# rampasek/DrVAE

Hardware: AMD Instinct MI355X
Metric: DrVAE ELBO training samples/sec (batch x L) (higher is better)
Workload: dtype f32; 1 GPU; cfg2: DrVAE bortezomib shape: 978 genes, z1=z3=100, enc-z1 800, dec-x 600, enc-z3/dec-z1 200, batch 150/GPU, L=2; global_batch=150, L=2, parallelism=dp1, launch=hipGraph replay, feed=resident, side_chain_cus=64, rccl_ranks=0, params=2321758

## Files before the change

### drvae_amd/csrc/rows.hip

```cpp
#include "dv_common.h"

namespace {

constexpr float kLog2Pi = 1.8378770664093453f;

inline int grid_for(int64_t work, int per_block, int cap = 4096) {
    int64_t b = (work + per_block - 1) / per_block;
    if (b < 1) b = 1;
    if (b > cap) b = cap;
    return (int)b;
}

__global__ __launch_bounds__(256) void colsum_kernel(const float* __restrict__ X, int64_t ldx, int M, int N,
                                                     float* __restrict__ out, float beta) {
    __shared__ float part[4][64];
    const int c = threadIdx.x & 63, rl = threadIdx.x >> 6;
    const int col = blockIdx.x * 64 + c;
    float s = 0.f;
    if (col < N) {
        const float* p = X + (int64_t)rl * ldx + col;
        const int64_t st = 4 * ldx;
        int m = rl;
        float a0 = 0.f, a1 = 0.f, a2 = 0.f, a3 = 0.f, a4 = 0.f, a5 = 0.f, a6 = 0.f, a7 = 0.f;
        for (; m + 28 < M; m += 32, p += 8 * st) {
            const float v0 = p[0], v1 = p[st], v2 = p[2 * st], v3 = p[3 * st];
            const float v4 = p[4 * st], v5 = p[5 * st], v6 = p[6 * st], v7 = p[7 * st];
            a0 += v0; a1 += v1; a2 += v2; a3 += v3;
            a4 += v4; a5 += v5; a6 += v6; a7 += v7;
        }
        s = ((a0 + a1) + (a2 + a3)) + ((a4 + a5) + (a6 + a7));
        for (; m < M; m += 4, p += st) s += p[0];
    }
    part[rl][c] = s;
    __syncthreads();
    if (rl == 0 && col < N) {
        s = part[0][c] + part[1][c] + part[2][c] + part[3][c];
        out[col] = (beta != 0.f ? beta * out[col] : 0.f) + s;
    }
}

__global__ void act_bwd_kernel(float* __restrict__ dY, int64_t ldd, const float* __restrict__ Y, int64_t ldy, int M,
                               int N, int split, int act0, int act1, float shift0, float shift1) {
    const int64_t total = (int64_t)M * N;
    for (int64_t e = blockIdx.x * (int64_t)blockDim.x + threadIdx.x; e < total; e += (int64_t)gridDim.x * blockDim.x) {
        const int m = (int)(e / N), n = (int)(e % N);
        const bool first = n < split;
        const float y = Y[(int64_t)m * ldy + n] - (first ? shift0 : shift1);
        dY[(int64_t)m * ldd + n] *= dv_dact_from_y(first ? act0 : act1, y);
    }
}

__global__ __launch_bounds__(256) void wn_scale_kernel(const float* __restrict__ W, int64_t ldw,
                                                       const float* __restrict__ g, int N, int K,
                                                       float* __restrict__ scale, float* __restrict__ norm) {
    const int lane = threadIdx.x & 63;
    const int row = blockIdx.x * 4 + (threadIdx.x >> 6);
    if (row >= N) return;
    const float* w = W + (int64_t)row * ldw;
    float s = 0.f;
    for (int k = lane; k < K; k += 64) s += w[k] * w[k];
    s = dv_wave_sum_all(s);
    if (lane == 0) {
        const float nrm = sqrtf(s);
        if (norm) norm[row] = nrm;
        scale[row] = g[row] / nrm;
    }
}

__global__ __launch_bounds__(256) void wn_bwd_kernel(const float* __restrict__ dWraw, int64_t ldr,
                                                     const float* __restrict__ W, int64_t ldw,
                                                     const float* __restrict__ g, const float* __restrict__ norm,
                                                     int N, int K, float* __restrict__ dW, int64_t ldd,
                                                     float* __restrict__ dg, float beta) {
    const int lane = threadIdx.x & 63;
    const int row = blockIdx.x * 4 + (threadIdx.x >> 6);
    if (row >= N) return;
    const float* w = W + (int64_t)row * ldw;
    const float* r = dWraw + (int64_t)row * ldr;
    float dot = 0.f;
    for (int k = lane; k < K; k += 64) dot += w[k] * r[k];
    dot = dv_wave_sum_all(dot);
    const float nrm = norm[row], gg = g[row];
    const float sc = gg / nrm, cw = dot * gg / (nrm * nrm * nrm);
    float* o = dW + (int64_t)row * ldd;
    for (int k = lane; k < K; k += 64) {
        const float v = sc * r[k] - cw * w[k];
        o[k] = (beta != 0.f ? beta * o[k] : 0.f) + v;
    }
    if (lane == 0) dg[row] = (beta != 0.f ? beta * dg[row] : 0.f) + dot / nrm;
}

__global__ void reparam_fwd_kernel(const float* __restrict__ mu, const float* __restrict__ sd, int64_t ldq,
                                   const int32_t* __restrict__ src_idx, int n, int reps, int Z,
                                   const float* __restrict__ eps, int64_t lde, int mode, float* __restrict__ out,
                                   int64_t ldo, const float* __restrict__ sub, int64_t lds,
                                   float* __restrict__ out2, int64_t ldo2, float* __restrict__ out3, int64_t ldo3,
                                   const int32_t* __restrict__ out3_idx) {
    const int64_t total = (int64_t)n * reps * Z;
    for (int64_t e = blockIdx.x * (int64_t)blockDim.x + threadIdx.x; e < total; e += (int64_t)gridDim.x * blockDim.x) {
        const int r = (int)(e / Z), d = (int)(e % Z);
        const int j = r % n;
        const int64_t qi = src_idx ? src_idx[j] : j;
        const float s = sd[qi * ldq + d];
        const float std_ = mode == DV_GAUSS_LOGVAR ? expf(0.5f * s) : s;
        const float z = eps[(int64_t)r * lde + d] * std_ + mu[qi * ldq + d];
        out[(int64_t)r * ldo + d] = z;
        if (out2) out2[(int64_t)r * ldo2 + d] = z - sub[(int64_t)r * lds + d];
        if (out3) {
            const int t = out3_idx[r];
            if (t >= 0) out3[(int64_t)t * ldo3 + d] = z;
        }
    }
}

__global__ void reparam_bwd_kernel(const float* __restrict__ dz, int64_t ldz, const float* __restrict__ eps,
                                   int64_t lde, const float* __restrict__ sd, int64_t ldq,
                                   const int32_t* __restrict__ src_idx, int n, int reps, int Z, int mode,
                                   float* __restrict__ dmu, float* __restrict__ dsd, int64_t lddq, float beta) {
    const int64_t total = (int64_t)n * Z;
    for (int64_t e = blockIdx.x * (int64_t)blockDim.x + threadIdx.x; e < total; e += (int64_t)gridDim.x * blockDim.x) {
        const int j = (int)(e / Z), d = (int)(e % Z);
        const int64_t qi = src_idx ? src_idx[j] : j;
        float a = 0.f, b = 0.f;
        for (int l = 0; l < reps; ++l) {
            const int64_t r = (int64_t)l * n + j;
            const float g = dz[r * ldz + d];
            a += g;
            b += g * eps[r * lde + d];
        }
        if (mode == DV_GAUSS_LOGVAR) b *= 0.5f * expf(0.5f * sd[qi * ldq + d]);
        float* pm = dmu + qi * lddq + d;
        float* ps = dsd + qi * lddq + d;
        *pm = (beta != 0.f ? beta * *pm : 0.f) + a;
        *ps = (beta != 0.f ? beta * *ps : 0.f) + b;
    }
}

#define DV_MAX_PARKED_GRID 512
typedef dv_wait ParkArgs;
typedef dv_bump CounterBump;

__device__ __forceinline__ void bump_counters(const CounterBump& bump) {
    for (int t = 0; t < 2; ++t) {
        if (bump.c[t] != nullptr) counter_add_words(bump.c[t], bump.n[t], bump.inc[t]);
    }
}

__device__ __forceinline__ float free_bits_gate(float c, float rv, float kl_min) {
    return c * (rv > kl_min ? 1.f : (rv == kl_min ? 0.5f : 0.f));
}

struct KlGrad {
    float gmq, gsq, gmp, gsp;
};
__device__ __forceinline__ KlGrad kl_grad_logvar(float mq, float sq, float mp, float sp) {
    const float dm = mq - mp, ivp = expf(-sp), vq = expf(sq);
    KlGrad g;
    g.gmq = dm * ivp;
    g.gsq = -0.5f * (1.f - vq * ivp);
    g.gmp = -g.gmq;
    g.gsp = -0.5f * (-1.f + (dm * dm + vq) * ivp);
    return g;
}

__global__ void reparam_bwd_seg_kernel(const float* __restrict__ dz, int64_t ldz, const float* __restrict__ eps,
                                       int64_t lde, const float* __restrict__ sd, int64_t ldq,
                                       const int32_t* __restrict__ seg_ptr, const int32_t* __restrict__ seg_rows,
                                       int nq, int Z, int mode, const float* __restrict__ extra, int64_t ldx,
                                       const int32_t* __restrict__ ex_ptr, const int32_t* __restrict__ ex_rows,
                                       float* __restrict__ dmu, float* __restrict__ dsd, int64_t lddq, float beta,
                                       CounterBump bump, const float* __restrict__ dz2, int64_t ldz2, int n2,
                                       ParkArgs park, dv_prior_kl pk) {
    park_block(park);
    if (blockIdx.x == 0 && threadIdx.x == 0) bump_counters(bump);
    const int64_t total = (int64_t)nq * Z;
    for (int64_t e = blockIdx.x * (int64_t)blockDim.x + threadIdx.x; e < total; e += (int64_t)gridDim.x * blockDim.x) {
        const int i = (int)(e / Z), d = (int)(e % Z);
        float a = 0.f, b = 0.f;
        for (int t = seg_ptr[i]; t < seg_ptr[i + 1]; ++t) {
            const int64_t r = seg_rows[t];
            float g = dz[r * ldz + d];
            if (r < n2) g += dz2[r * ldz2 + d];
            a += g;
            b += g * eps[r * lde + d];
        }
        if (mode == DV_GAUSS_LOGVAR) b *= 0.5f * expf(0.5f * sd[(int64_t)i * ldq + d]);
        if (extra) {
            for (int t = ex_ptr[i]; t < ex_ptr[i + 1]; ++t) {
                const int64_t r = ex_rows[t];
                a += extra[r * ldx + d];
                b += extra[r * ldx + Z + d];
            }
        }
        float* pm = dmu + (int64_t)i * lddq + d;
        float* ps = dsd + (int64_t)i * lddq + d;
        float vm = (beta != 0.f ? beta * *pm : 0.f) + a;
        float vs = (beta != 0.f ? beta * *ps : 0.f) + b;
        if (pk.coef != nullptr) {
            const float c = free_bits_gate(pk.coef[i], pk.raw[i], pk.kl_min);
            const float mq = pk.mu[(int64_t)i * pk.ld + d], vq = expf(sd[(int64_t)i * ldq + d]);
            vm += c * (mq * 1.f);
            vs += c * (-0.5f * (1.f - vq * 1.f));
        }
        *pm = vm;
        *ps = vs;
    }
}

struct Z2FArgs {
    const float* dz2f; int64_t ld_dz2f;
    const float* dzdec_pert; int64_t ld_pert;
    const int32_t* pair_slot;
    const float* eps; int64_t lde;
    const float* p2; int64_t ldp2;
    const float* q2; int64_t ldq2;
    const float* coef; const float* raw; float kl_min;
    const float* dz1b; int64_t ld_dz1b;
    float* dp2; int64_t ld_dp2;
    float* dz1; int64_t ld_dz1;
    float* dq2; int64_t ld_dq2;
    int L, B, Np, Z;
    const float* prior_coef; const float* prior_raw;
    float* kl_out; float* raw_out;
    const float* seg_src; int64_t ld_seg; const int32_t* seg_ptr; float seg_beta;
    float z1_dz2f;
};

__device__ __forceinline__ float kl_term(int mode, float mq, float sq, float mp, float sp) {
    const float dm = mq - mp;
    if (mode == DV_GAUSS_LOGVAR) return 1.f - sp + sq - (dm * dm + expf(sq)) / expf(sp);
    const float vq = sq * sq, vp = sp * sp;
    return 1.f - logf(vp) + logf(vq) - (dm * dm + vq) / vp;
}

struct Z2FElem {
    float mp, lp, gc, g, eps, z1, add;
};

__device__ __forceinline__ void z2f_load_own(const Z2FArgs& a, int64_t r, int64_t kr, int d, Z2FElem& e) {
    e.mp = a.p2[r * a.ldp2 + d];
    e.lp = a.p2[r * a.ldp2 + a.Z + d];
    e.g = (kr >= 0 && a.dzdec_pert) ? a.dzdec_pert[kr * a.ld_pert + d] : 0.f;
    e.eps = a.eps[r * a.lde + d];
    e.z1 = a.dz1[r * a.ld_dz1 + d];
}

__device__ __forceinline__ void z2f_load_side(const Z2FArgs& a, int64_t r, int d, int t0, int t1, Z2FElem& e) {
    e.gc = a.dz2f ? a.dz2f[r * a.ld_dz2f + d] : 0.f;
    e.g = e.gc + e.g;
    e.add = a.dz1b ? a.dz1b[r * a.ld_dz1b + d] : 0.f;
    if (a.seg_src != nullptr) {
        float s = 0.f;
        for (int t = t0; t < t1; ++t) s += a.seg_src[(int64_t)t * a.ld_seg + d];
        e.add += a.seg_beta * s;
    }
    if (a.z1_dz2f != 0.f) e.add += a.z1_dz2f * e.gc;
}

__device__ __forceinline__ void z2f_elem(const Z2FArgs& a, int64_t r, int d, bool pair, float c, float mq, float lq,
                                         const Z2FElem& e, float& gq_mu, float& gq_lv) {
    float dmu = e.g, dlv = e.g * e.eps * 0.5f * expf(0.5f * e.lp);
    if (pair) {
        const float dm = mq - e.mp, ivp = expf(-e.lp);
        const KlGrad k = kl_grad_logvar(mq, lq, e.mp, e.lp);
        gq_mu += c * dm * ivp;
        gq_lv += c * k.gsq;
        dmu += -c * dm * ivp;
        dlv += c * k.gsp;
    }
    a.dp2[r * a.ld_dp2 + d] = dmu;
    a.dp2[r * a.ld_dp2 + a.Z + d] = dlv;
    a.dz1[r * a.ld_dz1 + d] = e.z1 + (dmu + e.add);
}

struct Z2FRow {
    int jp;
    bool pair, own_kl, prior;
    float cpr, mq[2], lq[2], gm[2], gl[2];
};
struct Z2FPair {
    Z2FElem e[2][2];
    int t0[2], t1[2];
    float cf[2], rv[2];
};

__device__ __forceinline__ void z2f_row_begin(const Z2FArgs& a, int i, int lane, Z2FRow& w) {
    w.jp = a.pair_slot ? a.pair_slot[i] : -1;
    w.pair = w.jp >= 0;
    w.own_kl = w.pair && a.raw_out != nullptr;
    w.prior = w.pair && a.dq2 && a.prior_coef != nullptr;
    w.cpr = 0.f;
    if (w.prior)
        w.cpr = free_bits_gate(a.prior_coef[w.jp], a.prior_raw[w.jp], a.kl_min);
#pragma unroll
    for (int c = 0; c < 2; ++c) {
        const int d = lane + 64 * c;
        w.mq[c] = w.lq[c] = w.gm[c] = w.gl[c] = 0.f;
        if (w.pair && d < a.Z) {
            w.mq[c] = a.q2[(int64_t)w.jp * a.ldq2 + d];
            w.lq[c] = a.q2[(int64_t)w.jp * a.ldq2 + a.Z + d];
        }
    }
}

__device__ __forceinline__ void z2f_pair_own(const Z2FArgs& a, const Z2FRow& w, int i, int l0, int lane, Z2FPair& g) {
#pragma unroll
    for (int u = 0; u < 2; ++u) {
        g.t0[u] = g.t1[u] = 0;
        g.cf[u] = g.rv[u] = 0.f;
        if (l0 + u >= a.L) break;
        const int64_t r = (int64_t)(l0 + u) * a.B + i, kr = w.pair ? (int64_t)(l0 + u) * a.Np + w.jp : -1;
        if (a.seg_src != nullptr) {
            g.t0[u] = a.seg_ptr[r];
            g.t1[u] = a.seg_ptr[r + 1];
        }
        if (w.pair) g.cf[u] = a.coef[kr];
#pragma unroll
        for (int c = 0; c < 2; ++c)
            if (lane + 64 * c < a.Z) z2f_load_own(a, r, kr, lane + 64 * c, g.e[u][c]);
    }
    if (!w.own_kl) return;
#pragma unroll
    for (int u = 0; u < 2; ++u) {
        if (l0 + u >= a.L) break;
        float s = 0.f;
#pragma unroll
        for (int c = 0; c < 2; ++c)
            if (lane + 64 * c < a.Z) s += kl_term(DV_GAUSS_LOGVAR, w.mq[c], w.lq[c], g.e[u][c].mp, g.e[u][c].lp);
        g.rv[u] = -0.5f * dv_wave_sum_all(s);
        if (lane == 0) {
            const int64_t kr = (int64_t)(l0 + u) * a.Np + w.jp;
            a.raw_out[kr] = g.rv[u];
            a.kl_out[kr] = fmaxf(g.rv[u], a.kl_min);
        }
    }
}

__device__ __forceinline__ void z2f_pair_finish(const Z2FArgs& a, Z2FRow& w, int i, int l0, int lane, Z2FPair& g) {
#pragma unroll
    for (int u = 0; u < 2; ++u) {
        if (l0 + u >= a.L) break;
        const int64_t r = (int64_t)(l0 + u) * a.B + i;
        if (w.pair && !w.own_kl) g.rv[u] = a.raw[(int64_t)(l0 + u) * a.Np + w.jp];
#pragma unroll
        for (int c = 0; c < 2; ++c)
            if (lane + 64 * c < a.Z) z2f_load_side(a, r, lane + 64 * c, g.t0[u], g.t1[u], g.e[u][c]);
    }
#pragma unroll
    for (int u = 0; u < 2; ++u) {
        if (l0 + u >= a.L) break;
        const int64_t r = (int64_t)(l0 + u) * a.B + i;
        const float cg = w.pair ? free_bits_gate(g.cf[u], g.rv[u], a.kl_min) : 0.f;
#pragma unroll
        for (int c = 0; c < 2; ++c)
            if (lane + 64 * c < a.Z)
                z2f_elem(a, r, lane + 64 * c, w.pair, cg, w.mq[c], w.lq[c], g.e[u][c], w.gm[c], w.gl[c]);
    }
}
// ... 2408 lines not shown
                    for (; j + 3 < rl; j += 4) {
                        s0 += xr[j];
                        s1 += xr[j + 1];
                        s2 += xr[j + 2];
                        s3 += xr[j + 3];
                    }
                    for (; j < rl; ++j) s0 += xr[j];
                    q += t.w[r] * ((s0 + s1) + (s2 + s3));
                }
            } else {
                for (int i = threadIdx.x; i < t.n; i += kLossThreads) q += t.x[i];
            }
            ps[k] = q;
        }
    }
#pragma unroll
    for (int k = 0; k < DV_MAX_LOSS_TERMS; ++k) {
        if (k >= lt.n) continue;
        const float q = dv_wave_sum_all(ps[k]);
        if ((threadIdx.x & 63) == 0) part[k][threadIdx.x >> 6] = q;
    }
    __syncthreads();
    if (threadIdx.x == 0) {
        for (int i = 0; i < 8; ++i) acc[i] = 0.f;
        for (int k = 0; k < lt.n; ++k) {
            float q = 0.f;
            for (int w = 0; w < kLossThreads / 64; ++w) q += part[k][w];
            acc[lt.t[k].out] += lt.t[k].scale * q;
        }
    }
    if (threadIdx.x == 0) {
        if (!(flag != nullptr && lt.n == 0)) {
            acc[5] = we[0] * acc[0] + we[1] * acc[1] + we[2] * acc[2];
            float c = 0.f;
#pragma unroll
            for (int i = 0; i < 8; ++i) c += wc[i] * acc[i];
            acc[6] = c;
            bool bad = false;
            for (int i = 0; i < n_halt; ++i)
                bad = bad || __hip_atomic_load(halt + 2 * i, __ATOMIC_RELAXED, __HIP_MEMORY_SCOPE_AGENT) != 0;
            for (int i = 0; i < 8; ++i) loss[i] = bad ? __builtin_nanf("") : acc[i];
            if (accum != nullptr) {
#pragma unroll
                for (int i = 0; i < 8; ++i) accum[i] = ac[i] + (bad ? __builtin_nanf("") : acc[i]);
            }
        }
        bump_counters(bump);
    }
}

__global__ void axpby_kernel(const float* __restrict__ x, float a, float* __restrict__ y, float b, int64_t n) {
    for (int64_t i = blockIdx.x * (int64_t)blockDim.x + threadIdx.x; i < n; i += (int64_t)gridDim.x * blockDim.x)
        y[i] = a * x[i] + (b != 0.f ? b * y[i] : 0.f);
}

inline bool aligned16(const void* p) { return (reinterpret_cast<uintptr_t>(p) & 15) == 0; }

}

#define ST(s) static_cast<hipStream_t>(s)

static bool park_ok(const dv_wait* p) { return p == nullptr || p->flag == nullptr || (p->ctr && p->err && p->max_spins > 0); }
static bool bump_ok(const dv_bump* b) {
    return b == nullptr || ((!b->c[0] || b->n[0] == 1 || b->n[0] == 2) && (!b->c[1] || b->n[1] == 1 || b->n[1] == 2));
}

static int take_park(const dv_wait* in, int64_t grid, ParkArgs* park) {
    DV_REQUIRE(park_ok(in));
    *park = in ? *in : ParkArgs{};
    if (park->flag == nullptr) return DV_OK;
    DV_REQUIRE(grid > 0);
    return grid > DV_MAX_PARKED_GRID ? DV_ERR_UNSUPPORTED : DV_OK;
}

extern "C" int dv_colsum(const float* X, int64_t ldx, int32_t M, int32_t N, float* out, float beta,
                         dv_stream_t stream) {
    DV_REQUIRE(M >= 0 && N >= 0);
    if (N == 0) return DV_OK;
    DV_REQUIRE(X && out);
    hipLaunchKernelGGL(colsum_kernel, dim3((N + 63) / 64), dim3(256), 0, ST(stream), X, ldx, M, N, out, beta);
    DV_RETURN_LAUNCH();
}

extern "C" int dv_act_bwd(float* dY, int64_t ldd, const float* Y, int64_t ldy, int32_t M, int32_t N, int32_t split,
                          int32_t act0, int32_t act1, float shift0, float shift1, dv_stream_t stream) {
    DV_REQUIRE(M >= 0 && N >= 0);
    if (M == 0 || N == 0) return DV_OK;
    DV_REQUIRE(dY && Y);
    hipLaunchKernelGGL(act_bwd_kernel, dim3(grid_for((int64_t)M * N, 256)), dim3(256), 0, ST(stream), dY, ldd, Y,
                       ldy, M, N, split, act0, act1, shift0, shift1);
    DV_RETURN_LAUNCH();
}

extern "C" int dv_wn_scale(const float* W, int64_t ldw, const float* g, int32_t N, int32_t K, float* scale,
                           float* norm, dv_stream_t stream) {
    DV_REQUIRE(N >= 0 && K >= 0);
    if (N == 0) return DV_OK;
    DV_REQUIRE(W && g && scale);
    hipLaunchKernelGGL(wn_scale_kernel, dim3((N + 3) / 4), dim3(256), 0, ST(stream), W, ldw, g, N, K, scale, norm);
    DV_RETURN_LAUNCH();
}

extern "C" int dv_wn_bwd(const float* dWraw, int64_t ldr, const float* W, int64_t ldw, const float* g,
                         const float* norm, int32_t N, int32_t K, float* dW, int64_t ldd, float* dg, float beta,
                         dv_stream_t stream) {
    DV_REQUIRE(N >= 0 && K >= 0);
    if (N == 0) return DV_OK;
    DV_REQUIRE(dWraw && W && g && norm && dW && dg);
    hipLaunchKernelGGL(wn_bwd_kernel, dim3((N + 3) / 4), dim3(256), 0, ST(stream), dWraw, ldr, W, ldw, g, norm, N,
                       K, dW, ldd, dg, beta);
    DV_RETURN_LAUNCH();
}

extern "C" int dv_reparam_fwd(const float* mu, const float* sd, int64_t ldq, const int32_t* src_idx, int32_t n,
                              int32_t reps, int32_t Z, const float* eps, int64_t lde, int32_t mode, float* out,
                              int64_t ldo, const float* sub, int64_t lds, float* out2, int64_t ldo2, float* out3,
                              int64_t ldo3, const int32_t* out3_idx, dv_stream_t stream) {
    DV_REQUIRE(n >= 0 && reps >= 0 && Z >= 0);
    if (n == 0 || reps == 0 || Z == 0) return DV_OK;
    DV_REQUIRE(mu && sd && eps && out);
    DV_REQUIRE(out2 == nullptr || sub != nullptr);
    DV_REQUIRE(out3 == nullptr || out3_idx != nullptr);
    hipLaunchKernelGGL(reparam_fwd_kernel, dim3(grid_for((int64_t)n * reps * Z, 256)), dim3(256), 0, ST(stream), mu,
                       sd, ldq, src_idx, n, reps, Z, eps, lde, mode, out, ldo, sub, lds, out2, ldo2, out3, ldo3,
                       out3_idx);
    DV_RETURN_LAUNCH();
}

extern "C" int dv_reparam_bwd(const float* dz, int64_t ldz, const float* eps, int64_t lde, const float* sd,
                              int64_t ldq, const int32_t* src_idx, int32_t n, int32_t reps, int32_t Z, int32_t mode,
                              float* dmu, float* dsd, int64_t lddq, float beta, dv_stream_t stream) {
    DV_REQUIRE(n >= 0 && reps >= 0 && Z >= 0);
    if (n == 0 || Z == 0) return DV_OK;
    DV_REQUIRE(dz && eps && sd && dmu && dsd);
    hipLaunchKernelGGL(reparam_bwd_kernel, dim3(grid_for((int64_t)n * Z, 256)), dim3(256), 0, ST(stream), dz, ldz,
                       eps, lde, sd, ldq, src_idx, n, reps, Z, mode, dmu, dsd, lddq, beta);
    DV_RETURN_LAUNCH();
}

extern "C" int dv_reparam_bwd_seg(const float* dz, int64_t ldz, const float* eps, int64_t lde, const float* sd,
                                  int64_t ldq, const int32_t* seg_ptr, const int32_t* seg_rows, int32_t nq,
                                  int32_t Z, int32_t mode, const float* extra, int64_t ldx, const int32_t* ex_ptr,
                                  const int32_t* ex_rows, float* dmu, float* dsd, int64_t lddq, float beta,
                                  const dv_bump* bump_in, const dv_seg_add* add, const dv_wait* park_in,
                                  const dv_prior_kl* prior, dv_stream_t stream) {
    DV_REQUIRE(bump_ok(bump_in));
    DV_REQUIRE(prior == nullptr || prior->coef == nullptr || (prior->raw && prior->mu && mode == DV_GAUSS_LOGVAR));
    const dv_prior_kl pk = prior ? *prior : dv_prior_kl{};
    const CounterBump bump = bump_in ? *bump_in : CounterBump{};
    DV_REQUIRE(nq >= 0 && Z >= 0);
    DV_REQUIRE(!(bump.c[0] || bump.c[1]) || (nq > 0 && Z > 0));
    DV_REQUIRE(add == nullptr || add->n == 0 || (add->dz && add->n > 0));
    ParkArgs park;
    if (int rc = take_park(park_in, nq > 0 && Z > 0 ? grid_for((int64_t)nq * Z, 256) : 0, &park)) return rc;
    if (nq == 0 || Z == 0) return DV_OK;
    DV_REQUIRE(dz && eps && sd && seg_ptr && seg_rows && dmu && dsd);
    DV_REQUIRE(extra == nullptr || (ex_ptr && ex_rows));
    hipLaunchKernelGGL(reparam_bwd_seg_kernel, dim3(grid_for((int64_t)nq * Z, 256)), dim3(256), 0, ST(stream), dz,
                       ldz, eps, lde, sd, ldq, seg_ptr, seg_rows, nq, Z, mode, extra, ldx, ex_ptr, ex_rows, dmu, dsd,
                       lddq, beta, bump, add ? add->dz : nullptr, add ? add->ld : 0, add ? add->n : 0, park, pk);
    DV_RETURN_LAUNCH();
}

extern "C" int dv_z2f_post_bwd(const dv_z2f_desc* dsc, const dv_wait* park_in, dv_stream_t stream) {
    DV_REQUIRE(dsc != nullptr);
    const dv_z2f_desc& d = *dsc;
    DV_REQUIRE(d.L >= 0 && d.B >= 0 && d.Np >= 0 && d.Z >= 0);
    ParkArgs park;
    if (int rc = take_park(park_in, d.L > 0 && d.B > 0 && d.Z > 0 ? grid_for(d.B, 4) : 0, &park)) return rc;
    if (d.L == 0 || d.B == 0 || d.Z == 0) return DV_OK;
    DV_REQUIRE(d.eps && d.p2 && d.dp2 && d.dz1);
    DV_REQUIRE((d.kl_out == nullptr) == (d.raw_out == nullptr));
    DV_REQUIRE(d.Np == 0 || (d.pair_slot && d.q2 && d.coef && (d.raw || d.raw_out)));
    DV_REQUIRE((d.prior_coef == nullptr) == (d.prior_raw == nullptr));
    DV_REQUIRE((d.seg_src == nullptr) == (d.seg_ptr == nullptr));
    Z2FArgs a{d.dz2f, d.ld_dz2f, d.dzdec_pert, d.ld_pert, d.Np ? d.pair_slot : nullptr, d.eps, d.lde, d.p2, d.ldp2,
              d.q2, d.ldq2, d.coef, d.raw, d.kl_min, d.dz1b, d.ld_dz1b, d.dp2, d.ld_dp2, d.dz1, d.ld_dz1, d.dq2,
              d.ld_dq2, d.L, d.B, d.Np, d.Z, d.Np ? d.prior_coef : nullptr, d.Np ? d.prior_raw : nullptr,
              d.Np ? d.kl_out : nullptr, d.Np ? d.raw_out : nullptr, d.seg_src, d.ld_seg, d.seg_ptr, d.seg_beta,
              d.dz2f ? d.z1_dz2f : 0.f};
    if (d.Z <= 128)
        hipLaunchKernelGGL(z2f_post_bwd_kernel, dim3(grid_for(d.B, 4)), dim3(256), 0, ST(stream), a, park);
    else
        hipLaunchKernelGGL(z2f_post_bwd_wide_kernel, dim3(grid_for(d.B, 4)), dim3(256), 0, ST(stream), a, park);
    DV_RETURN_LAUNCH();
}

extern "C" int dv_kl_rows_fwd(const dv_kl_rows_desc* dsc, const dv_wait* park_in, dv_stream_t stream) {
    DV_REQUIRE(dsc != nullptr);
    const dv_kl_rows_desc& d = *dsc;
    DV_REQUIRE(d.n >= 0 && d.reps >= 0 && d.Z >= 0);
    DV_REQUIRE((d.mu2 == nullptr) == (d.sd2 == nullptr) && (d.mu2 == nullptr || d.Z2 >= 0));
    ParkArgs park;
    if (int rc = take_park(park_in, d.n > 0 && d.reps > 0 ? grid_for((int64_t)d.n * d.reps, 4) : 0, &park)) return rc;
    if (d.n == 0 || d.reps == 0) return DV_OK;
    DV_REQUIRE(d.mu_q && d.sd_q && d.out);
    DV_REQUIRE((d.mu_p == nullptr) == (d.sd_p == nullptr));
    DV_REQUIRE(d.zout == nullptr || d.eps != nullptr);
    KlArgs a{d.mu_q, d.sd_q, d.ldq, d.qidx, d.mu_p, d.sd_p, d.ldp, d.pidx, d.prior_mu, d.prior_sd, d.n, d.reps, d.Z, d.mode};
    hipLaunchKernelGGL(kl_rows_fwd_kernel, dim3(grid_for((int64_t)d.n * d.reps, 4)), dim3(256), 0, ST(stream), a,
                       d.free_bits, d.kl_min, d.raw_out, d.out, d.add, d.eps, d.lde, d.zout, d.ldz, park, d.mu2, d.sd2,
                       d.ld2, d.Z2, d.raw2_out);
    DV_RETURN_LAUNCH();
}

static int kl_fwd_of(const dv_kl_rows_desc& d, KlFwd& f) {
    DV_REQUIRE(d.n >= 0 && d.reps >= 0 && d.Z >= 0 && d.mu_q && d.sd_q && d.out);
    DV_REQUIRE((d.mu_p == nullptr) == (d.sd_p == nullptr));
    DV_REQUIRE(d.zout == nullptr && d.eps == nullptr && d.mu2 == nullptr && d.sd2 == nullptr);
    f = KlFwd{KlArgs{d.mu_q, d.sd_q, d.ldq, d.qidx, d.mu_p, d.sd_p, d.ldp, d.pidx, d.prior_mu, d.prior_sd, d.n, d.reps, d.Z,
                     d.mode},
              d.free_bits, d.kl_min, d.raw_out, d.out, d.add};
    return DV_OK;
}

extern "C" int dv_kl_rows_fwd_pair(const dv_kl_rows_desc* d1, const dv_kl_rows_desc* d2, dv_stream_t stream) {
    DV_REQUIRE(d1 != nullptr && d2 != nullptr);
    KlFwd a, b;
    int rc = kl_fwd_of(*d1, a);
    if (rc != DV_OK) return rc;
    rc = kl_fwd_of(*d2, b);
    if (rc != DV_OK) return rc;
    const int64_t ba = ((int64_t)d1->n * d1->reps + 3) / 4, bb = ((int64_t)d2->n * d2->reps + 3) / 4;
    if (ba + bb == 0) return DV_OK;
    if (ba + bb > 0x7fffffff) return DV_ERR_UNSUPPORTED;
    hipLaunchKernelGGL(kl_rows_fwd_pair_kernel, dim3((unsigned)(ba + bb)), dim3(256), 0, ST(stream), a, b, (int)ba);
    DV_RETURN_LAUNCH();
}

extern "C" int dv_kl_rows_bwd(const dv_kl_rows_desc* dsc, const dv_kl_rows_grad* grad, dv_stream_t stream) {
    DV_REQUIRE(dsc != nullptr && grad != nullptr);
    const dv_kl_rows_desc& d = *dsc;
    const dv_kl_rows_grad& g = *grad;
    DV_REQUIRE(d.n >= 0 && d.reps >= 0 && d.Z >= 0);
    if (d.n == 0 || d.reps == 0 || d.Z == 0) return DV_OK;
    DV_REQUIRE(g.coef && d.mu_q && d.sd_q && g.dq_mu && g.dq_sd);
    DV_REQUIRE(!d.free_bits || d.raw_out != nullptr);
    DV_REQUIRE((d.mu_p == nullptr) == (d.sd_p == nullptr));
    DV_REQUIRE((g.dp_mu == nullptr) == (g.dp_sd == nullptr));
    DV_REQUIRE(g.dp_mu == nullptr || d.mu_p != nullptr);
    DV_REQUIRE(g.dz == nullptr || d.eps != nullptr);
    KlArgs a{d.mu_q, d.sd_q, d.ldq, d.qidx, d.mu_p, d.sd_p, d.ldp, d.pidx, d.prior_mu, d.prior_sd, d.n, d.reps, d.Z, d.mode};
    hipLaunchKernelGGL(kl_rows_bwd_kernel, dim3(grid_for((int64_t)d.n * d.reps * d.Z, 256)), dim3(256), 0, ST(stream), a,
                       g.coef, (const float*)d.raw_out, d.free_bits, d.kl_min, g.dq_mu, g.dq_sd, g.lddq, g.dp_mu, g.dp_sd,
                       g.lddp, g.beta, g.dz, g.ldz, d.eps, d.lde);
    DV_RETURN_LAUNCH();
}

extern "C" int dv_gauss_nll_rows_fwd(const float* x, int64_t ldx, const int32_t* xidx, const float* mu,
                                     const float* sd, int64_t ldp, int32_t M, int32_t X, int32_t mode, float* out,
                                     const float* bias_mu, const float* bias_sd, float sd_shift, dv_stream_t stream) {
    DV_REQUIRE(M >= 0 && X >= 0);
    if (M == 0) return DV_OK;
    DV_REQUIRE(x && mu && sd && out && ((bias_mu == nullptr) == (bias_sd == nullptr)));
    DV_REQUIRE(bias_mu == nullptr || mode == DV_GAUSS_SIGMA);
    const bool v4 = aligned16(x) && aligned16(mu) && aligned16(sd) && (ldx % 4 == 0) && (ldp % 4 == 0);
    auto a8 = [](const void* p) { return (reinterpret_cast<uintptr_t>(p) & 7) == 0; };
    const bool v2 = a8(x) && a8(mu) && a8(sd) && (ldx % 2 == 0) && (ldp % 2 == 0) && (!bias_mu || (a8(bias_mu) && a8(bias_sd)));
    const dim3 grid(grid_for(M, 4, 8192)), block(256);
#define DV_NLL_FWD(VEC, RAW)                                                                                             \
    hipLaunchKernelGGL((nll_rows_fwd_kernel<VEC, RAW>), grid, block, 0, ST(stream), x, ldx, xidx, mu, sd, ldp, M, X, mode, \
                       out, bias_mu, bias_sd, sd_shift)
    if (bias_mu) {
        if (v4) DV_NLL_FWD(4, true);
        else if (v2) DV_NLL_FWD(2, true);
        else DV_NLL_FWD(1, true);
    } else {
        if (v4) DV_NLL_FWD(4, false);
        else if (v2) DV_NLL_FWD(2, false);
        else DV_NLL_FWD(1, false);
    }
#undef DV_NLL_FWD
    DV_RETURN_LAUNCH();
}

extern "C" int dv_gauss_nll_rows_fwdbwd(const float* coef, const float* x, int64_t ldx, const int32_t* xidx,
                                        const float* mu, const float* sd, int64_t ldp, int32_t M, int32_t X,
                                        int32_t mode, int32_t sd_act, float sd_shift, float* out, float* dmu,
                                        float* dsd, int64_t ldd, const float* bias_mu, const float* bias_sd,
                                        dv_stream_t stream) {
    DV_REQUIRE(M >= 0 && X >= 0);
    if (M == 0) return DV_OK;
    DV_REQUIRE(coef && x && mu && sd && out && dmu && dsd && ((bias_mu == nullptr) == (bias_sd == nullptr)));
    auto a8 = [](const void* p) { return (reinterpret_cast<uintptr_t>(p) & 7) == 0; };
    const bool v2 = a8(x) && a8(mu) && a8(sd) && a8(dmu) && a8(dsd) && (ldx % 2 == 0) && (ldp % 2 == 0) && (ldd % 2 == 0);
    const dim3 grid(M < 16384 ? M : 16384), block(256);
    auto a16 = [](const void* p) { return (reinterpret_cast<uintptr_t>(p) & 15) == 0; };
    if (bias_mu && mode == DV_GAUSS_SIGMA && sd_act == DV_ACT_SOFTPLUS && X % 4 == 0 && ldx % 4 == 0 && ldp % 4 == 0 &&
        ldd % 4 == 0 && a16(x) && a16(mu) && a16(sd) && a16(dmu) && a16(dsd) && a16(bias_mu) && a16(bias_sd)) {
        hipLaunchKernelGGL(nll_rows_raw_sp_kernel, grid, block, 0, ST(stream), coef, x, ldx, xidx, mu, sd, ldp, M, X,
                           sd_shift, out, dmu, dsd, ldd, bias_mu, bias_sd);
        DV_RETURN_LAUNCH();
    }
    if (v2)
        hipLaunchKernelGGL(nll_rows_fwdbwd_kernel<true>, grid, block, 0, ST(stream), coef, x, ldx, xidx, mu, sd, ldp, M,
                           X, mode, sd_act, sd_shift, out, dmu, dsd, ldd, bias_mu, bias_sd);
    else
        hipLaunchKernelGGL(nll_rows_fwdbwd_kernel<false>, grid, block, 0, ST(stream), coef, x, ldx, xidx, mu, sd, ldp,
                           M, X, mode, sd_act, sd_shift, out, dmu, dsd, ldd, bias_mu, bias_sd);
    DV_RETURN_LAUNCH();
}

extern "C" int dv_gauss_nll_rows_raw_cs(const dv_nll_raw_cs_desc* dsc, dv_stream_t stream) {
    DV_REQUIRE(dsc != nullptr);
    const dv_nll_raw_cs_desc& d = *dsc;
    DV_REQUIRE(d.M >= 0 && d.X >= 4 && d.X % 4 == 0);
    if (d.M == 0) return DV_OK;
    const bool fwd_only = d.dmu == nullptr;
    DV_REQUIRE(d.x && d.mu && d.sd && d.out_part && d.bias_mu && d.bias_sd);
    DV_REQUIRE(fwd_only ? (d.dsd == nullptr && d.ws == nullptr) : (d.coef && d.dsd && d.ws));
    auto a16 = [](const void* p) { return (reinterpret_cast<uintptr_t>(p) & 15) == 0; };
    DV_REQUIRE(a16(d.x) && a16(d.mu) && a16(d.sd) && a16(d.bias_mu) && a16(d.bias_sd));
    DV_REQUIRE(d.ldx % 4 == 0 && d.ldp % 4 == 0);
// ... 655 lines not shown
```

Before: 1.724 million samples/s.

## Restructure segmented reparam backward to wave-per-row with register-batched gathers

Remaps the segmented reparameterization backward kernel so each wave owns one query row and 64 latent columns instead of flat element indexing. Segment pointers, the prior coefficient and raw values are fetched once per wave and broadcast with readlane. For short segments (up to 8 rows) the row indices are loaded in one shot and all gathers are issued before accumulation, exposing memory-level parallelism. This adds register pressure, a fallback loop for long segments, a new grid computation that must respect parked-grid limits, and explicit no-contract helpers to keep the arithmetic bit-identical.

Result: no change. 1.740 million samples/s (median of 6 runs) (+0.9%).

```diff
diff --git a/drvae_amd/csrc/rows.hip b/drvae_amd/csrc/rows.hip
--- a/drvae_amd/csrc/rows.hip
+++ b/drvae_amd/csrc/rows.hip
@@ -163,47 +163,142 @@
     return g;
 }
 
-__global__ void reparam_bwd_seg_kernel(const float* __restrict__ dz, int64_t ldz, const float* __restrict__ eps,
-                                       int64_t lde, const float* __restrict__ sd, int64_t ldq,
-                                       const int32_t* __restrict__ seg_ptr, const int32_t* __restrict__ seg_rows,
-                                       int nq, int Z, int mode, const float* __restrict__ extra, int64_t ldx,
-                                       const int32_t* __restrict__ ex_ptr, const int32_t* __restrict__ ex_rows,
-                                       float* __restrict__ dmu, float* __restrict__ dsd, int64_t lddq, float beta,
-                                       CounterBump bump, const float* __restrict__ dz2, int64_t ldz2, int n2,
-                                       ParkArgs park, dv_prior_kl pk) {
+__device__ __forceinline__ void seg_sample(float& a, float& b, float g, float g2, bool has2, float e) {
+#pragma clang fp contract(off)
+    if (has2) g = g + g2;
+    a = a + g;
+    b = b + g * e;
+}
+__device__ __forceinline__ void seg_scale(float& b, float sd) {
+#pragma clang fp contract(off)
+    b = b * (0.5f * expf(0.5f * sd));
+}
+__device__ __forceinline__ void seg_extra(float& a, float& b, float xa, float xb) {
+#pragma clang fp contract(off)
+    a = a + xa;
+    b = b + xb;
+}
+__device__ __forceinline__ void seg_finish(float& vm, float& vs, float a, float b, float beta, float om, float os,
+                                           bool prior, float c, float mq, float sd) {
+#pragma clang fp contract(off)
+    vm = (beta != 0.f ? beta * om : 0.f) + a;
+    vs = (beta != 0.f ? beta * os : 0.f) + b;
+    if (prior) {
+        vm = __builtin_fmaf(c, mq, vm);
+        vs = __builtin_fmaf(c, -0.5f * (1.f - expf(sd)), vs);
+    }
+}
+
+struct SegArgs {
+    const float* dz; int64_t ldz;
+    const float* eps; int64_t lde;
+    const float* sd; int64_t ldq;
+    const int32_t* seg_ptr; const int32_t* seg_rows;
+    int nq, Z, mode;
+    const float* extra; int64_t ldx;
+    const int32_t* ex_ptr; const int32_t* ex_rows;
+    float* dmu; float* dsd; int64_t lddq;
+    float beta;
+    const float* dz2; int64_t ldz2; int n2;
+};
+
+__device__ __forceinline__ void seg_loop_sums(const SegArgs& s, int t0, int t1, int x0, int x1, int d, float sdv, float& a,
+                                              float& b) {
+    a = 0.f;
+    b = 0.f;
+    for (int t = t0; t < t1; ++t) {
+        const int64_t r = s.seg_rows[t];
+        const bool has2 = r < s.n2;
+        seg_sample(a, b, s.dz[r * s.ldz + d], has2 ? s.dz2[r * s.ldz2 + d] : 0.f, has2, s.eps[r * s.lde + d]);
+    }
+    if (s.mode == DV_GAUSS_LOGVAR) seg_scale(b, sdv);
+    for (int t = x0; t < x1; ++t) {
+        const int64_t r = s.ex_rows[t];
+        seg_extra(a, b, s.extra[r * s.ldx + d], s.extra[r * s.ldx + s.Z + d]);
+    }
+}
+
+constexpr int kSegRegs = 8;
+
+__global__ __launch_bounds__(256) void reparam_bwd_seg_kernel(SegArgs s, int gx, CounterBump bump, ParkArgs park,
+                                                              dv_prior_kl pk) {
     park_block(park);
     if (blockIdx.x == 0 && threadIdx.x == 0) bump_counters(bump);
-    const int64_t total = (int64_t)nq * Z;
-    for (int64_t e = blockIdx.x * (int64_t)blockDim.x + threadIdx.x; e < total; e += (int64_t)gridDim.x * blockDim.x) {
-        const int i = (int)(e / Z), d = (int)(e % Z);
+    const int lane = threadIdx.x & 63;
+    const int wave = __builtin_amdgcn_readfirstlane(threadIdx.x >> 6);
+    const bool logvar = s.mode == DV_GAUSS_LOGVAR, prior = pk.coef != nullptr, old = s.beta != 0.f;
+    int bx = blockIdx.x, d0 = 0;
+    while (bx >= gx) {
+        bx -= gx;
+        d0 += 64;
+    }
+    const int d = d0 + lane;
+    const int dl = min(d, s.Z - 1);
+    for (int i = bx * 4 + wave; i < s.nq; i += gx * 4) {
+        const void* wp = nullptr;
+        if (lane < 2) wp = s.seg_ptr + i + lane;
+        if ((lane == 2 || lane == 3) && s.extra != nullptr) wp = s.ex_ptr + i + lane - 2;
+        if (lane == 4 && prior) wp = pk.coef + i;
+        if (lane == 5 && prior) wp = pk.raw + i;
+        int word = 0;
+        if (wp != nullptr) __builtin_memcpy(&word, __builtin_assume_aligned(wp, 4), 4);
+        float sdv = 0.f, om = 0.f, os = 0.f, mq = 0.f;
+        if (logvar || prior) sdv = s.sd[(int64_t)i * s.ldq + dl];
+        if (old) {
+            om = s.dmu[(int64_t)i * s.lddq + dl];
+            os = s.dsd[(int64_t)i * s.lddq + dl];
+        }
+        if (prior) mq = pk.mu[(int64_t)i * pk.ld + dl];
+        const int t0 = __builtin_amdgcn_readlane(word, 0), t1 = __builtin_amdgcn_readlane(word, 1);
+        const int x0 = __builtin_amdgcn_readlane(word, 2), x1 = __builtin_amdgcn_readlane(word, 3);
+        const float cf = __int_as_float(__builtin_amdgcn_readlane(word, 4));
+        const float rw = __int_as_float(__builtin_amdgcn_readlane(word, 5));
+        const int ns = t1 - t0, nx = x1 - x0;
         float a = 0.f, b = 0.f;
-        for (int t = seg_ptr[i]; t < seg_ptr[i + 1]; ++t) {
-            const int64_t r = seg_rows[t];
-            float g = dz[r * ldz + d];
-            if (r < n2) g += dz2[r * ldz2 + d];
-            a += g;
-            b += g * eps[r * lde + d];
-        }
-        if (mode == DV_GAUSS_LOGVAR) b *= 0.5f * expf(0.5f * sd[(int64_t)i * ldq + d]);
-        if (extra) {
-            for (int t = ex_ptr[i]; t < ex_ptr[i + 1]; ++t) {
-                const int64_t r = ex_rows[t];
-                a += extra[r * ldx + d];
-                b += extra[r * ldx + Z + d];
-            }
-        }
-        float* pm = dmu + (int64_t)i * lddq + d;
-        float* ps = dsd + (int64_t)i * lddq + d;
-        float vm = (beta != 0.f ? beta * *pm : 0.f) + a;
-        float vs = (beta != 0.f ? beta * *ps : 0.f) + b;
-        if (pk.coef != nullptr) {
-            const float c = free_bits_gate(pk.coef[i], pk.raw[i], pk.kl_min);
-            const float mq = pk.mu[(int64_t)i * pk.ld + d], vq = expf(sd[(int64_t)i * ldq + d]);
-            vm += c * (mq * 1.f);
-            vs += c * (-0.5f * (1.f - vq * 1.f));
-        }
-        *pm = vm;
-        *ps = vs;
+        if (ns <= kSegRegs && nx <= kSegRegs) {
+            int rowsv = 0;
+            {
+                const int k = lane & 31;
+                const bool isx = lane >= 32;
+                const int32_t* list = isx ? s.ex_rows + x0 : s.seg_rows + t0;
+                if (k < (isx ? nx : ns)) rowsv = list[k];
+            }
+            const int r0 = __builtin_amdgcn_readlane(rowsv, 0);
+            float gz[kSegRegs], g2[kSegRegs], ep[kSegRegs], xa[kSegRegs], xb[kSegRegs];
+#pragma unroll
+            for (int k = 0; k < kSegRegs; ++k) {
+                if (k < ns) {
+                    const int64_t r = k == 0 ? r0 : __builtin_amdgcn_readlane(rowsv, k);
+                    gz[k] = s.dz[r * s.ldz + dl];
+                    ep[k] = s.eps[r * s.lde + dl];
+                    if (r < s.n2) g2[k] = s.dz2[r * s.ldz2 + dl];
+                }
+            }
+#pragma unroll
+            for (int k = 0; k < kSegRegs; ++k) {
+                if (k < nx) {
+                    const int64_t r = __builtin_amdgcn_readlane(rowsv, 32 + k);
+                    xa[k] = s.extra[r * s.ldx + dl];
+                    xb[k] = s.extra[r * s.ldx + s.Z + dl];
+                }
+            }
+#pragma unroll
+            for (int k = 0; k < kSegRegs; ++k)
+                if (k < ns) seg_sample(a, b, gz[k], g2[k], __builtin_amdgcn_readlane(rowsv, k) < s.n2, ep[k]);
+            if (logvar) seg_scale(b, sdv);
+#pragma unroll
+            for (int k = 0; k < kSegRegs; ++k)
+                if (k < nx) seg_extra(a, b, xa[k], xb[k]);
+        } else {
+            seg_loop_sums(s, t0, t1, x0, x1, dl, sdv, a, b);
+        }
+        if (d < s.Z) {
+            const float cg = prior ? free_bits_gate(cf, rw, pk.kl_min) : 0.f;
+            float vm, vs;
+            seg_finish(vm, vs, a, b, s.beta, om, os, prior, cg, mq, sdv);
+            s.dmu[(int64_t)i * s.lddq + d] = vm;
+            s.dsd[(int64_t)i * s.lddq + d] = vs;
+        }
     }
 }
 
@@ -2918,13 +3013,17 @@
     DV_REQUIRE(!(bump.c[0] || bump.c[1]) || (nq > 0 && Z > 0));
     DV_REQUIRE(add == nullptr || add->n == 0 || (add->dz && add->n > 0));
     ParkArgs park;
-    if (int rc = take_park(park_in, nq > 0 && Z > 0 ? grid_for((int64_t)nq * Z, 256) : 0, &park)) return rc;
+    const bool parked = park_in != nullptr && park_in->flag != nullptr;
+    const int nblk = (Z + 63) / 64;
+    const int gx = grid_for(nq, 4, std::max(1, (parked ? DV_MAX_PARKED_GRID : 4096) / std::max(nblk, 1)));
+    DV_REQUIRE(!parked || nblk <= DV_MAX_PARKED_GRID);
+    if (int rc = take_park(park_in, nq > 0 && Z > 0 ? gx * nblk : 0, &park)) return rc;
     if (nq == 0 || Z == 0) return DV_OK;
     DV_REQUIRE(dz && eps && sd && seg_ptr && seg_rows && dmu && dsd);
     DV_REQUIRE(extra == nullptr || (ex_ptr && ex_rows));
-    hipLaunchKernelGGL(reparam_bwd_seg_kernel, dim3(grid_for((int64_t)nq * Z, 256)), dim3(256), 0, ST(stream), dz,
-                       ldz, eps, lde, sd, ldq, seg_ptr, seg_rows, nq, Z, mode, extra, ldx, ex_ptr, ex_rows, dmu, dsd,
-                       lddq, beta, bump, add ? add->dz : nullptr, add ? add->ld : 0, add ? add->n : 0, park, pk);
+    const SegArgs sa{dz, ldz, eps, lde, sd, ldq, seg_ptr, seg_rows, nq, Z, mode, extra, ldx, ex_ptr, ex_rows, dmu, dsd, lddq,
+                     beta, add ? add->dz : nullptr, add ? add->ld : 0, add ? add->n : 0};
+    hipLaunchKernelGGL(reparam_bwd_seg_kernel, dim3(gx * nblk), dim3(256), 0, ST(stream), sa, gx, bump, park, pk);
     DV_RETURN_LAUNCH();
 }
 
```
